# vlad17/runlmc

Hardware: AMD Instinct MI355X
Metric: kronecker_toeplitz_mvms_per_sec (higher is better)
Workload: dtype f64; 1 GPU; c5 synthetic D=10 Q=5 R=1 m=100000 (grid 100004, L=204800) N=128 probes/GPU, batch=129 vectors/step, K_UU product, kernel family rbf; kern=rbf, D=10, Q=5, m=100004, L=204800, batch=129, parallelism=probe-shard x1

## Files before the change

### runlmc_amd/csrc/rl_gridop.hip

```cpp
#include "rl_host.h"

static thread_local std::string g_err;

int fail(int code, const std::string& msg) {
    g_err = msg;
    return code;
}

extern "C" const char* rl_last_error(void) { return g_err.c_str(); }
extern "C" const char* rl_backend(void) { return RL_BACKEND_NAME; }
extern "C" int rl_abi_version(void) { return RL_ABI_VERSION; }
extern "C" int rl_device_count(int* count) {
    if (!count) return fail(RL_EINVAL, "count is NULL");
    RL_HIP(hipGetDeviceCount(count));
    return RL_OK;
}

void trace_once(const char* what) {
    static const bool on = getenv("RUNLMC_TRACE") != nullptr;
    if (!on) return;
    static std::vector<std::string> seen;
    for (const std::string& s : seen)
        if (s == what) return;
    seen.push_back(what);
    fprintf(stderr, "[runlmc] %s\n", what);
}

bool first_on_device(unsigned long long* seen) {
    int dev = 0;
    (void)hipGetDevice(&dev);
    const unsigned long long bit = 1ull << (dev & 63);
    if (*seen & bit) return false;
    *seen |= bit;
    return true;
}

RlKnobs read_knobs() {
    RlKnobs k;
    const char* dbg = getenv("RUNLMC_DEBUG");
    const bool debug = dbg != nullptr && dbg[0] != '\0' && dbg[0] != '0';
    auto ignored = [](const char* n) {
        static std::vector<std::string> told;
        if (std::find(told.begin(), told.end(), std::string(n)) == told.end()) {
            told.push_back(n);
            fprintf(stderr, "runlmc_hip: %s is a debug switch and is ignored without RUNLMC_DEBUG=1\n", n);
        }
    };
    auto user_flag = [](const char* n) { return getenv(n) != nullptr; };
    auto user_num = [](const char* n, long long dflt) {
        const char* e = getenv(n);
        return e ? atoll(e) : dflt;
    };
    auto flag = [&](const char* n) {
        if (getenv(n) == nullptr) return false;
        if (!debug) ignored(n);
        return debug;
    };
    auto num = [&](const char* n, long long dflt) {
        const char* e = getenv(n);
        if (e == nullptr) return dflt;
        if (!debug) ignored(n);
        return debug ? atoll(e) : dflt;
    };
    k.pow2_only = user_flag("RUNLMC_POW2_ONLY");
    k.chunk_mb = (int)num("RUNLMC_CHUNK_MB", 0);
    k.two_streams = (int)num("RUNLMC_TWO_STREAMS", -1);
    k.affine = (int)num("RUNLMC_AFFINE", -1);
    k.affine_kb = (int)num("RUNLMC_AFFINE_KB", 0);
    k.affine_max_kb = (int)num("RUNLMC_AFFINE_MAX_KB", 2048);
    k.no_v1p = flag("RUNLMC_NO_V1P");
    k.v1p_min = (int)num("RUNLMC_V1P_MIN", 0);
    k.no_lowrank = flag("RUNLMC_NO_LOWRANK");
    k.no_filter = flag("RUNLMC_NO_FILTER");
    k.no_lr_bound = flag("RUNLMC_NO_LR_BOUND");
    k.sf_carries1 = flag("RUNLMC_SF_CARRIES1");
    k.sf_scan2 = flag("RUNLMC_SF_SCAN2");
    k.poly_round = flag("RUNLMC_POLY_ROUND");
    k.no_poly_round = flag("RUNLMC_NO_POLY_ROUND");
    k.lr_min = num("RUNLMC_LR_MIN", -1);
    k.staged_wt = flag("RUNLMC_STAGED_WT");
    k.no_staged_wt = flag("RUNLMC_NO_STAGED_WT");
    k.no_w_poly = flag("RUNLMC_NO_W_POLY");
    k.no_rp = flag("RUNLMC_NO_RP");
    k.rp_stagger = (int)num("RUNLMC_RP_STAGGER", 7);
    k.no_lr_small = flag("RUNLMC_NO_LR_SMALL");
    k.no_precond_approx = flag("RUNLMC_NO_PRECOND_APPROX");
    k.no_precond_hi = flag("RUNLMC_NO_PRECOND_HI");
    k.precond_hi_passes = flag("RUNLMC_PRECOND_HI_PASSES");
    k.no_precond_hi_mixed = flag("RUNLMC_NO_PRECOND_HI_MIXED");
    k.precond_hi_min = num("RUNLMC_PRECOND_HI_MIN", 100000);
    k.precond_hi_rank = (int)num("RUNLMC_PRECOND_HI_RANK", 192);
    k.precond_hi_use = (int)num("RUNLMC_PRECOND_HI_USE", 0);
    k.rp_fly = (int)num("RUNLMC_RP_FLY", 1);
    k.no_rp_small = flag("RUNLMC_NO_RP_SMALL");
    k.no_rp_fuse = flag("RUNLMC_NO_RP_FUSE");
    k.rp_pfuse = !flag("RUNLMC_NO_RP_PFUSE");
    k.w_pfuse = !flag("RUNLMC_NO_W_PFUSE");
    k.rp_runlen = (int)num("RUNLMC_RP_RUNLEN", 0);
    k.w_poly_rmax = std::min(36, (int)num("RUNLMC_W_POLY_RMAX", 32));
    k.no_sort = flag("RUNLMC_NO_SORT");
    k.ws_cache_mb = user_num("RUNLMC_WS_CACHE_MB", -1);
    k.solver_maxblk = (int)num("RUNLMC_SOLVER_MAXBLK", 0);
    k.no_fuse_w = flag("RUNLMC_NO_FUSE_W");
    k.no_fuse_wt = flag("RUNLMC_NO_FUSE_WT");
    k.no_graph = flag("RUNLMC_NO_GRAPH");
#if defined(RL_EMU)
    k.minres_v1 = flag("RUNLMC_MINRES_V1");
#endif
    return k;
}

static int ilog2(int x) {
    int l = 0;
    while ((1 << l) < x) ++l;
    return l;
}

static FftPlan make_plan(int n) {
    FftPlan p;
    p.n = n;
    p.npass = 0;
    for (int i = 0; i < RL_MAX_PASSES; ++i) p.radix[i] = 1;
    int rem = n;
    for (int odd : {3, 5})
        while (rem % odd == 0 && p.npass < 2) {
            p.radix[p.npass++] = odd;
            rem /= odd;
        }
    const int fixed[7][4] = {{8, 8, 0, 0},     {16, 16, 0, 0},   {64, 8, 8, 0},
                             {128, 8, 16, 0},  {256, 16, 16, 0}, {512, 8, 8, 8},
                             {1024, 8, 8, 16}};
    for (const auto& f : fixed)
        if (f[0] == rem) {
            for (int i = 1; i < 4 && f[i]; ++i) p.radix[p.npass++] = f[i];
            return p;
        }
    while (rem > 1) {
        int r = 8;
        while (rem % r) r /= 2;
        p.radix[p.npass++] = r;
        rem /= r;
    }
    return p;
}

static bool make_plan_rows3(int n, FftPlan* p) {
    int ra, rb;
    switch (n) {
        case 128: ra = 8; rb = 8; break;
        case 256: ra = 16; rb = 8; break;
        case 512: ra = 16; rb = 16; break;
        default: return false;
    }
    p->n = n;
    p->npass = 3;
    for (int i = 0; i < RL_MAX_PASSES; ++i) p->radix[i] = 1;
    p->radix[0] = ra;
    p->radix[1] = rb;
    p->radix[2] = 2;
    return true;
}

static int fused_code(const FftPlan& p) {
    if (p.npass < 2 || p.npass > 4) return 0;
    const int ra = p.radix[0], rb = p.radix[p.npass - 1];
    const int code = ra * 100 + rb;
    switch (code) {
        case 808: case 816: case 1616: return p.n >= 64 ? code : 0;
// ... 983 lines not shown
        for (int n = 0; n < m; ++n) {
            prev[n] = cur[n];
            cur[n] = nxt[n] / bj;
        }
    }
    RL_TRY(upload(&g->lr_phiJ, phiJ));
    RL_TRY(upload(&g->lr_beta, beta));
    RL_TRY(upload(&g->lr_nu, nu));
    g->lr_hnu = nu;
    return RL_OK;
}

static int lr_steps(const rl_gridop* g, int nrows, int R) {
    const int slots = (g->m + 1) / 2;
    if (slots <= 64 * RL_LR_T) return std::max(4, ((slots + 63) / 64 + 3) / 4 * 4);
    const int rowblocks = (nrows + RL_LR_ROWS(R) - 1) / RL_LR_ROWS(R);
    const double resident = 2.0 * RL_LR_CUS;
    int best = RL_LR_T;
    double best_cost = 1e300;
    for (int steps = RL_LR_T; steps <= 8 * RL_LR_T; steps *= 2) {
        const int chunks = ((g->m + 1) / 2 + 64 * steps - 1) / (64 * steps);
        const double rounds = std::ceil((double)chunks * rowblocks / resident);
        const double cost = rounds * (steps + 8);
        if (cost < best_cost * 0.97) {
            best_cost = cost;
            best = steps;
        }
        if (chunks == 1) break;
    }
    return best;
}
static int lr_nchunks_max(const rl_gridop* g) {
    return ((g->m + 1) / 2 + 64 * RL_LR_T - 1) / (64 * RL_LR_T);
}
static size_t lr_part_need(const rl_gridop* g, int nvec) {
    return (size_t)lr_nchunks_max(g) * nvec * g->D * RL_LR_RMAX;
}
int lr_reserve(rl_gridop* g, int nvec) {
    const size_t rows = (size_t)nvec * g->D;
    const size_t need_part = lr_part_need(g, nvec), need_z = rows * RL_LR_RMAX;
    if (g->lr_part_cap < need_part) {
        if (g->lr_part) RL_HIP(hipFree(g->lr_part));
        g->lr_part = nullptr;
        g->lr_part_cap = 0;
        RL_HIP(hipMalloc((void**)&g->lr_part, need_part * sizeof(double)));
        g->lr_part_cap = need_part;
    }
    if (g->lr_zhat_cap < need_z) {
        if (g->lr_zhat) RL_HIP(hipFree(g->lr_zhat));
        g->lr_zhat = nullptr;
        g->lr_zhat_cap = 0;
        RL_HIP(hipMalloc((void**)&g->lr_zhat, need_z * sizeof(double)));
        g->lr_zhat_cap = need_z;
    }
    return RL_OK;
}

static size_t lr_min_elements(const rl_gridop* g) {
    return g->kn.lr_min >= 0 ? (size_t)g->kn.lr_min : (size_t)1 << 20;
}

template <int R>
static int lr_project(rl_gridop* g, const double* X, int nrows, hipStream_t st,
                      double* part = nullptr) {
    const int steps = lr_steps(g, nrows, R);
    const int chunks = ((g->m + 1) / 2 + 64 * steps - 1) / (64 * steps);
    RL_LAUNCH((k_lr_project<R>), dim3(chunks, (nrows + RL_LR_ROWS(R) - 1) / RL_LR_ROWS(R)),
              dim3(64 * RL_LR_WAVES), (size_t)RL_LR_WAVES * R * 65 * sizeof(double), st, X, nrows,
              g->m, (const double*)g->lr_beta, steps, part != nullptr ? part : g->lr_part);
    return chunks;
}
template <int R>
static void lr_mix(rl_gridop* g, const double* part, int chunks, int nvec, int Q, const double* Cq,
                   const double* Bq, double* zhat, hipStream_t st) {
    int split3 = 0;
    const size_t mix_lds = lr_mix_lds(g->D, R, Q, &split3);
    RL_LAUNCH(k_lr_mix, dim3(nvec), dim3(RL_LR_MIXT), mix_lds, st, part, chunks, nvec, g->D, R, Q,
              Cq, Bq, (const double*)g->lr_nu, zhat, (const int*)nullptr, split3);
}
template <int R>
static void lr_expand(rl_gridop* g, const double* zhat, int nrows, double* Y, int accumulate,
                      hipStream_t st) {
    const int per_cu = 8;
    const int nbx = ((g->m + 1) / 2 + 255) / 256;
    int rpb = 16;
    if ((size_t)nbx * ((nrows + 15) / 16) < (size_t)2 * per_cu * RL_LR_CUS) {
        const int nby = std::max(1, std::min(nrows, per_cu * RL_LR_CUS / nbx));
        rpb = (nrows + nby - 1) / nby;
    }
    if (accumulate)
        RL_LAUNCH((k_lr_expand<R, true>), dim3(nbx, (nrows + rpb - 1) / rpb), dim3(256), 0,
                  st, zhat, nrows, g->m, (const double*)g->lr_beta, rpb, Y);
    else
        RL_LAUNCH((k_lr_expand<R, false>), dim3(nbx, (nrows + rpb - 1) / rpb), dim3(256), 0,
                  st, zhat, nrows, g->m, (const double*)g->lr_beta, rpb, Y);
}
template <int R>
static void lr_launch(rl_gridop* g, const double* X, double* Y, int nvec, int Q, const double* Cq,
                      const double* Bq, hipStream_t st, int accumulate = 0) {
    const int nrows = nvec * g->D;
    const bool deferred = g->defer_expand && !accumulate && R <= g->kn.w_poly_rmax;
    const int chunks = lr_project<R>(g, X, nrows, st);
    lr_mix<R>(g, g->lr_part, chunks, nvec, Q, Cq, Bq, g->lr_zhat, st);
    if (deferred) {
        g->expand_deferred = true;
        return;
    }
    lr_expand<R>(g, g->lr_zhat, nrows, Y, accumulate, st);
}

static int lr_apply(rl_gridop* g, const double* X, double* Y, int nvec, int q0, int Q,
                    const double* Bq, hipStream_t st) {
    const double* Cq = g->lr_C + (size_t)q0 * g->lr_r * g->lr_r;
    switch (g->lr_r) {
        case 24: lr_launch<24>(g, X, Y, nvec, Q, Cq, Bq, st); break;
        case 32: lr_launch<32>(g, X, Y, nvec, Q, Cq, Bq, st); break;
        case 36: lr_launch<36>(g, X, Y, nvec, Q, Cq, Bq, st); break;
        case 40: lr_launch<40>(g, X, Y, nvec, Q, Cq, Bq, st); break;
        case 48: lr_launch<48>(g, X, Y, nvec, Q, Cq, Bq, st); break;
        default: return fail(RL_EINVAL, "low-rank path: bad basis size");
    }
    RL_HIP(hipGetLastError());
    return RL_OK;
}

static int lr_apply_compact(rl_gridop* g, const double* X, double* Y, int nvec, hipStream_t st) {
    switch (g->lr_r) {
        case 24: lr_launch<24>(g, X, Y, nvec, g->lr_np, g->lr_Cc, g->lr_Bc, st, 1); break;
        case 32: lr_launch<32>(g, X, Y, nvec, g->lr_np, g->lr_Cc, g->lr_Bc, st, 1); break;
        case 36: lr_launch<36>(g, X, Y, nvec, g->lr_np, g->lr_Cc, g->lr_Bc, st, 1); break;
        case 40: lr_launch<40>(g, X, Y, nvec, g->lr_np, g->lr_Cc, g->lr_Bc, st, 1); break;
        case 48: lr_launch<48>(g, X, Y, nvec, g->lr_np, g->lr_Cc, g->lr_Bc, st, 1); break;
        default: return fail(RL_EINVAL, "low-rank path: bad basis size");
    }
    RL_HIP(hipGetLastError());
    return RL_OK;
}

static int mvm_with_mix(rl_gridop* g, const MixParams& mp, const double* X, double* Y, int nvec,
                        hipStream_t stream);

struct SfFit {
    int deg = 0;
    long double ah = 0.0L;
    long double c[4] = {0.0L, 0.0L, 0.0L, 0.0L};
};

static bool sf_check(const double* t, int m, const SfFit& f, long double tot) {
    const long double budget = (long double)RL_SF_TOL * tot, rho = expl(-f.ah);
    long double err = 0.0L, pw = 1.0L;
    for (int i = 0; i < m; ++i) {
        if ((i & 255) == 0) pw = expl(-f.ah * i);
        const long double model = (f.c[0] + (f.c[1] + (f.c[2] + f.c[3] * i) * i) * i) * pw;
        err += fabsl((long double)t[i] - model);
        if (!(err <= budget)) return false;
        pw *= rho;
    }
    return true;
}

static bool sf_detect(const double* t, int m, SfFit* fit) {
    if (m < 8) return false;
    long double tot = 0.0L;
    double amax = 0.0;
    int imax = 0;
    for (int i = 0; i < m; ++i) {
        if (!std::isfinite(t[i])) return false;
        const double a = std::fabs(t[i]);
        tot += a;
        if (a > amax) {
            amax = a;
            imax = i;
        }
    }
    if (amax == 0.0) return false;
    int below = -1;
    for (int i = imax; i < m; ++i)
        if (std::fabs(t[i]) <= 0.6 * amax) {
// ... 1102 lines not shown
```

### runlmc_amd/csrc/rl_host.h

```cpp
#pragma once
#include "../../include/runlmc_hip.h"

#include <algorithm>
#include <cmath>
#include <cstdio>
#include <cstdlib>
#include <cstring>
#include <functional>
#include <string>
#include <thread>
#include <vector>

#include "rl_kernels.h"
#include "rl_kernels2.h"
#include "rl_kernels3.h"
#include "rl_lowrank.h"
#include "rl_rowpoly.h"
#include "rl_filter.h"

#define RL_MAX_D 16

int fail(int code, const std::string& msg);
#define RL_HIP(expr)                                                                   \
    do {                                                                               \
        hipError_t e_ = (expr);                                                        \
        if (e_ != hipSuccess)                                                          \
            return fail(RL_EHIP, std::string(#expr) + ": " + hipGetErrorString(e_));   \
    } while (0)

#define RL_TRY(expr)              \
    do {                          \
        int rc_ = (expr);         \
        if (rc_ != RL_OK) return rc_; \
    } while (0)


void trace_once(const char* what);
bool first_on_device(unsigned long long* seen);

struct RlKnobs {
    bool pow2_only = false;
    int chunk_mb = 0;
    int two_streams = -1;
    int affine = -1;
    int affine_kb = 0;
    int affine_max_kb = 2048;
    bool no_v1p = false;
    int v1p_min = 0;
    bool no_lowrank = false;
    bool no_filter = false;
    bool sf_scan2 = false;
    bool sf_carries1 = false;
    bool no_lr_bound = false;
    bool poly_round = false;
    bool no_poly_round = false;
    long long lr_min = -1;
    bool staged_wt = false;
    bool no_staged_wt = false;
    bool no_w_poly = false;
    bool no_rp = false;
    int rp_stagger = 7;
    int rp_runlen = 0;
    bool no_rp_small = false;
    bool rp_pfuse = true;
    bool w_pfuse = true;
    bool no_rp_fuse = false;
    bool no_lr_small = false;
    bool no_precond_approx = false;
    long long precond_hi_min = 100000;
    int precond_hi_use = 0;
    int precond_hi_rank = 192;
    bool no_precond_hi_mixed = false;
    bool precond_hi_passes = false;
    bool no_precond_hi = false;
    int rp_fly = 1;
    int w_poly_rmax = 32;
    bool no_sort = false;
    long long ws_cache_mb = -1;
    int solver_maxblk = 0;
    bool no_fuse_w = false;
    bool no_fuse_wt = false;
    bool no_graph = false;
    bool minres_v1 = false;
};
RlKnobs read_knobs();

template <class T>
static int upload(T** dev, const std::vector<T>& host) {
    RL_HIP(hipMalloc((void**)dev, std::max<size_t>(host.size(), 1) * sizeof(T)));
    if (!host.empty())
        RL_HIP(hipMemcpy(*dev, host.data(), host.size() * sizeof(T), hipMemcpyHostToDevice));
    return RL_OK;
}

static const size_t kLdsSoft = 76 * 1024;
static const size_t kLdsHard = 156 * 1024;

struct rl_gridop {
    RlKnobs kn;
    int device = 0;
    int D = 0, m = 0, L = 0, N1 = 0, N2 = 0;
    Geom geo{0, 0, 0};
    int colsA = 0;
    int rowsB = 0;
    int rowsS = 0;
    int code1 = 0, code2 = 0;
    bool v2 = false;
    bool rows3 = false;
    bool lr_try = false;
    bool lr_ok = false;
    bool lr_round_try = false;
    bool wide = false;
    rl_gridop* child = nullptr;
    double* wide_B = nullptr;
    double* wide_Z = nullptr;
    size_t wide_Z_cap = 0;
    bool defer_expand = false;
    bool expand_deferred = false;
    int lr_rejects = 0;
    int lr_skip = 0;
    double* lr_stat = nullptr;
    bool lr_dirty = false;
    std::vector<double> lr_A, lr_W, lr_kap;
    std::vector<int> lr_Qi;
    bool lr_bypass = false;
    int lr_r = 0;
    int lr_rank_hint = 0;
    size_t lr_min = 0;
    double* lr_beta = nullptr;
    double* lr_nu = nullptr;
    double* lr_phiJ = nullptr;
    double* lr_C = nullptr;
    double* lr_M = nullptr;
    std::vector<double> lr_hC;
    double* lr_spart = nullptr;
    size_t lr_spart_cap = 0;
    double* lr_Cx = nullptr;
    double* lr_Mf = nullptr;
    size_t lr_Mf_cap = 0;
    bool lr_Mf_ok = false;
    std::vector<double> lr_hB;
    std::vector<double> lr_hnu;
    unsigned long long param_ver = 0;
    double* lr_B = nullptr;
    double* lr_eye = nullptr;
    double* lr_part = nullptr;
    size_t lr_part_cap = 0;
    double* lr_zhat = nullptr;
    size_t lr_zhat_cap = 0;
    double* lr_scr = nullptr;
// ... 245 lines not shown
```

### runlmc_amd/csrc/rl_lowrank.h

```cpp
#pragma once
#include "rl_device.h"

#define RL_LR_RMAX 48
#define RL_LR_T 32
#define RL_LR_WAVES 4
#define RL_LR_CUS 256
#define RL_LR_RB(R) ((R) <= 24 ? 4 : 2)
#define RL_LR_G(R) ((R) <= 24 ? 2 : 4)
#define RL_LR_ROWS(R) (RL_LR_RB(R) * RL_LR_WAVES)
#if defined(RL_EMU)
#define RL_LR_PROJECT_ATTR
#define RL_LR_UNIFORM(x) (x)
#else
#define RL_LR_PROJECT_ATTR __attribute__((amdgpu_waves_per_eu(2)))
#define RL_LR_UNIFORM(x) __builtin_amdgcn_readfirstlane(x)
#endif
#define RL_LR_TOL 2e-13

__device__ __forceinline__ int lr_slots(int m) { return (m + 1) / 2; }
__device__ __forceinline__ double lr_point(int n, int m) {
    return m > 1 ? fma(2.0 / (double)(m - 1), (double)n, -1.0) : 0.0;
}

template <int R>
// ... 149 lines not shown
        const double* z = Z + b * r;
        double s = 0.0;
        for (int j = 0; j < r; ++j) s = fma(c[j], z[j], s);
        W[e] = s;
    }
    __syncthreads();
    if (!split3) {
        for (int e = tid; e < Dr; e += nthr) {
            const int a = e / r, i = e - a * r;
            double s = 0.0;
            for (int q = 0; q < Q; ++q) {
                const double* bq = Bq + ((size_t)q * D + a) * D;
                for (int b = 0; b < D; ++b) s = fma(bq[b], W[(q * D + b) * r + i], s);
            }
            Zhat[(size_t)v * Dr + e] = nu[i] * s;
        }
        return;
    }
    for (int e = tid; e < Q * Dr; e += nthr) {
        const int q = e / Dr, rem = e - q * Dr;
        const int a = rem / r, i = rem - a * r;
        const double* bq = Bq + ((size_t)q * D + a) * D;
        double s = 0.0;
        for (int b = 0; b < D; ++b) s = fma(bq[b], W[(q * D + b) * r + i], s);
        S[e] = s;
    }
    __syncthreads();
    for (int e = tid; e < Dr; e += nthr) {
        double s = 0.0;
        for (int q = 0; q < Q; ++q) s += S[q * Dr + e];
        Zhat[(size_t)v * Dr + e] = nu[e % r] * s;
    }
}

template <int R, bool ACC>
__global__ void __launch_bounds__(256)
k_lr_expand(const double* __restrict__ Zhat, int nrows, int m, const double* __restrict__ beta,
            int rows_per_block, double* __restrict__ Y) {
    const int slots = lr_slots(m);
    const int lin = blockIdx.y * gridDim.x + blockIdx.x;
    const int bx = lin / gridDim.y, by = lin - bx * gridDim.y;
    const int n = bx * 256 + threadIdx.x;
    const int nc = n < slots ? n : slots - 1;
    const int mir = m - 1 - nc;
    const bool live = n < slots, pair = live && mir != nc;
    const int row0 = by * rows_per_block;
    const int row1 = row0 + rows_per_block < nrows ? row0 + rows_per_block : nrows;
    const double s = lr_point(nc, m);
    double p[R];
    {
        double qm = 0.0, q = 1.0;
#pragma unroll
        for (int j = 0; j < R; ++j) {
            p[j] = q;
            const double qn = fma(s, q, -beta[j] * qm);
            qm = q;
            q = qn;
        }
    }
    for (int row = row0; row < row1; ++row) {
        const double* z = Zhat + (size_t)row * R;
        double zz[R];
#pragma unroll
        for (int j = 0; j < R; ++j) zz[j] = z[j];
#if !defined(RL_EMU)
        __builtin_amdgcn_sched_barrier(0);
#endif
        double ev = 0.0, od = 0.0;
#pragma unroll
        for (int j = 0; j + 1 < R; j += 2) {
            ev = fma(zz[j], p[j], ev);
            od = fma(zz[j + 1], p[j + 1], od);
        }
        double* y0 = Y + (size_t)row * m + nc;
        double* y1 = Y + (size_t)row * m + mir;
        double o0 = 0.0, o1 = 0.0;
        if constexpr (ACC) {
            o0 = *y0;
            o1 = *y1;
        }
        if (live) *y0 = (ev + od) + o0;
        if (pair) *y1 = (ev - od) + o1;
    }
}

#define RL_LR_SMALL_MAX 32768
#define RL_LR_SMALL_WG 256
#define RL_LR_SU 4
#define RL_LR_SMP 32
static inline int lr_small_nseg(int m) {
    const int slots = (m + 1) / 2;
    int nseg = (slots + RL_LR_SMALL_WG * RL_LR_SU - 1) / (RL_LR_SMALL_WG * RL_LR_SU);
    return nseg < 1 ? 1 : (nseg > 16 ? 16 : nseg);
}
template <int R>
__global__ void __launch_bounds__(RL_LR_SMALL_WG)
k_lr_small_project(const double* __restrict__ X, int D, int m, int nseg, const double* __restrict__ beta,
                   double* __restrict__ part) {
    RL_SMEM(smem);
    double* red = reinterpret_cast<double*>(smem);
    double* wsum = red + (size_t)4 * R * 65;
    const int tid = threadIdx.x, lane = tid & 63, wave = tid >> 6;
    const int b = blockIdx.x / nseg, sg = blockIdx.x - b * nseg, v = blockIdx.y;
    const int slots = lr_slots(m), seglen = (slots + nseg - 1) / nseg;
    const int n0 = sg * seglen, n1 = n0 + seglen < slots ? n0 + seglen : slots;
    const double* xb = X + ((size_t)v * D + b) * m;
    double acc[R];
#pragma unroll
    for (int j = 0; j < R; ++j) acc[j] = 0.0;
    for (int nb = n0 + tid; nb < n1; nb += RL_LR_SMALL_WG * RL_LR_SU) {
        double s[RL_LR_SU], q[RL_LR_SU], qm[RL_LR_SU], xe[RL_LR_SU], xo[RL_LR_SU];
#pragma unroll
        for (int u = 0; u < RL_LR_SU; ++u) {
            const int n = nb + RL_LR_SMALL_WG * u;
            const bool live = n < n1;
            const int nc = live ? n : n1 - 1, mir = m - 1 - nc;
            const double x0 = live ? xb[nc] : 0.0, x1 = live && mir != nc ? xb[mir] : 0.0;
            xe[u] = x0 + x1;
            xo[u] = x0 - x1;
            s[u] = lr_point(nc, m);
            q[u] = 1.0;
            qm[u] = 0.0;
        }
#pragma unroll
        for (int j = 0; j < R; ++j) {
            const double nbj = -beta[j];
#pragma unroll
            for (int u = 0; u < RL_LR_SU; ++u) {
                acc[j] = fma(q[u], (j & 1) ? xo[u] : xe[u], acc[j]);
                const double qn = fma(s[u], q[u], nbj * qm[u]);
                qm[u] = q[u];
                q[u] = qn;
            }
        }
    }
#pragma unroll
    for (int j = 0; j < R; ++j) red[((size_t)wave * R + j) * 65 + lane] = acc[j];
    __syncthreads();
    if (tid < 4 * R) {
        const double* src = red + (size_t)tid * 65;
        double s0 = 0.0, s1 = 0.0, s2 = 0.0, s3 = 0.0;
#pragma unroll 4
        for (int l = 0; l < 64; l += 4) {
            s0 += src[l];
            s1 += src[l + 1];
            s2 += src[l + 2];
            s3 += src[l + 3];
        }
        wsum[tid] = (s0 + s1) + (s2 + s3);
    }
    __syncthreads();
    if (tid < R)
        part[(((size_t)v * D + b) * nseg + sg) * R + tid] =
            (wsum[tid] + wsum[R + tid]) + (wsum[2 * R + tid] + wsum[3 * R + tid]);
}
static inline size_t lr_small_project_lds(int R) { return ((size_t)4 * R * 65 + 4 * R) * sizeof(double); }
static inline size_t lr_small_expand_lds(int D, int R) { return ((size_t)D * R + 256 + R) * sizeof(double); }

template <int R>
__global__ void __launch_bounds__(RL_LR_SMALL_WG)
k_lr_small_expand(const double* __restrict__ part, int D, int m, int nseg, const double* __restrict__ beta,
                  const double* __restrict__ Mf, double* __restrict__ Y) {
    RL_SMEM(smem);
    double* Z = reinterpret_cast<double*>(smem);
    double* P = Z + (size_t)D * R;
    double* Zh = P + 256;
// ... 259 lines not shown
```

### runlmc_amd/csrc/rl_sample.hip

```cpp
#include "rl_host.h"
#include "rl_sample.h"

#include <complex>

typedef std::complex<double> cd;

static const int kSmpTile = 4096;
static const int kSmpAxis2d = 2048;
static const long long kSmpMaxLen = 1ll << 22;

struct rl_sampler {
    rl_gridop* g = nullptr;
    int device = 0, D = 0, m = 0, m1 = 0, m2 = 0;
    bool set = false;
    int Q = 0, nemb = 0, npoly = 0, poly_rank = 0;
    long long zlen = 0;
    int N1 = 0, N2 = 0;
    bool one_launch = false;
    int cols = 1, rows = 1, K1 = 0;
    FftPlan plan1, plan2;
    cplx *tw1 = nullptr, *tw2 = nullptr, *twlo = nullptr;
    int *freq1 = nullptr, *pos1 = nullptr, *freq2 = nullptr;
    int* eC = nullptr;
    int* efoff = nullptr;
// ... 252 lines not shown
        RL_TRY(upload(&h->eC, eC));
        RL_TRY(upload(&h->efoff, efoff));
        RL_TRY(upload(&h->ezoff, ezoff));
        const int n1 = N1s, n2 = twod ? N2s : 1;
        const size_t ext_len = (size_t)(n1 / 2 + 1) * (twod ? n2 / 2 + 1 : 1);
        std::vector<double> slam((size_t)nemb * Ltot);
        h->h_lam.assign((size_t)nemb * Ltot, 0.0);
        int e = 0;
        for (int q = 0; q < Q; ++q) {
            if (forms[q] != 0) {
                if (clipped) clipped[q] = 0.0;
                continue;
            }
            const std::vector<double> lam = smp_spectrum(ext_rows + (size_t)e * ext_len, n1, n2);
            long double neg = 0.0L, tot = 0.0L;
            for (long long w = 0; w < Ltot; ++w) {
                const double v = lam[w];
                tot += std::fabs(v);
                if (v < 0.0) neg += -v;
                slam[(size_t)e * Ltot + w] = v > 0.0 ? std::sqrt(v / (double)Ltot) : 0.0;
                h->h_lam[(size_t)e * Ltot + w] = v > 0.0 ? v : 0.0;
            }
            if (clipped) clipped[q] = tot > 0.0L ? (double)(neg / tot) : 0.0;
            ++e;
        }
        RL_TRY(upload(&h->slam, slam));
        h->one_launch = !twod && Ltot <= RL_SAMPLER_LDS_MAX;
        if (h->one_launch) {
            h->N1 = (int)Ltot;
            h->N2 = 1;
        } else if (twod) {
            h->N1 = N1s;
            h->N2 = N2s;
        } else {
            int odd = 1;
            (void)smp_length_ok(Ltot, &odd);
            const long long P = Ltot / odd;
            int n2p = 1;
            while (2 * n2p <= kSmpTile && P % (2 * n2p) == 0 && Ltot / (2 * n2p) >= 16) n2p *= 2;
            h->N2 = n2p;
            h->N1 = (int)(Ltot / n2p);
            if (h->N1 > kSmpTile || h->N2 > kSmpTile || h->N1 < 1)
                return fail(RL_ELIMIT, "rl_sampler_set: embedding length has no two-pass split");
        }
        h->plan1 = smp_plan(h->N1);
        const std::vector<int> f1 = smp_pos_to_freq(h->plan1);
        RL_TRY(upload(&h->freq1, f1));
        RL_TRY(upload(&h->pos1, smp_invert(f1)));
        RL_TRY(upload(&h->tw1, smp_unity(h->N1, 1, h->N1)));
        if (!h->one_launch) {
            h->plan2 = smp_plan(h->N2);
            RL_TRY(upload(&h->freq2, smp_pos_to_freq(h->plan2)));
            RL_TRY(upload(&h->tw2, smp_unity(h->N2, 1, h->N2)));
            RL_TRY(upload(&h->twlo, smp_unity(h->N2, 1, Ltot)));
            h->cols = std::max(1, std::min(16, kSmpTile / h->N1));
            h->rows = std::max(1, std::min(16, kSmpTile / h->N2));
            while (h->rows > 1 && (long long)h->N2 * (h->rows | 1) > kSmpTile) --h->rows;
            h->K1 = twod ? h->m1 : std::min(h->N1, h->m);
        }
    }
    if (npoly) {
        RL_TRY(upload(&h->pC, pC));
        RL_TRY(upload(&h->pfoff, pfoff));
        RL_TRY(upload(&h->pzoff, pzoff));
        std::vector<double> hG(poly_sqrt, poly_sqrt + (size_t)npoly * poly_rank * poly_rank);
        RL_TRY(upload(&h->G, hG));
    }
    *zlen = h->zlen;
    h->set = true;
    return RL_OK;
}

extern "C" int rl_sampler_spectrum_host(const rl_sampler* h, int q, double* out) {
    if (!h || !out) return fail(RL_EINVAL, "rl_sampler_spectrum_host: NULL argument");
    if (!h->set || q < 0 || q >= h->Q || h->emb_of[q] < 0)
        return fail(RL_EINVAL, "rl_sampler_spectrum_host: not a row in the embedding form");
    const size_t Ltot = (size_t)h->N1 * h->N2;
    memcpy(out, h->h_lam.data() + (size_t)h->emb_of[q] * Ltot, Ltot * sizeof(double));
    return RL_OK;
}

template <int R>
static void smp_expand(rl_sampler* h, double* U, int nrows, bool accumulate, hipStream_t st) {
    const int slots = (h->m + 1) / 2, nbx = (slots + 255) / 256;
    const int nby = std::max(1, std::min(nrows, 4 * RL_LR_CUS / nbx));
    const int rpb = (nrows + nby - 1) / nby;
    const dim3 grid(nbx, (nrows + rpb - 1) / rpb);
    if (accumulate)
        RL_LAUNCH((k_lr_expand<R, true>), grid, dim3(256), 0, st, (const double*)h->zhat, nrows, h->m,
                  (const double*)h->g->lr_beta, rpb, U);
    else
        RL_LAUNCH((k_lr_expand<R, false>), grid, dim3(256), 0, st, (const double*)h->zhat, nrows, h->m,
                  (const double*)h->g->lr_beta, rpb, U);
}

extern "C" int rl_sampler_draw(rl_sampler* h, const double* Z, double* U, int nsamp, void* stream) {
    if (!h || !Z || !U) return fail(RL_EINVAL, "rl_sampler_draw: NULL argument");
    if (!h->set) return fail(RL_EINVAL, "rl_sampler_draw: no parameters (rl_sampler_set)");
    if (nsamp < 0) return fail(RL_EINVAL, "rl_sampler_draw: nsamp < 0");
    if (nsamp == 0) return RL_OK;
    const int npairs = (nsamp + 1) / 2;
    if (npairs > 65535) return fail(RL_ELIMIT, "rl_sampler_draw: at most 131070 draws per call");
    RL_HIP(hipSetDevice(h->device));
    hipStream_t st = (hipStream_t)stream;
    const int D = h->D;
    if (h->nemb) {
        SmpRows R{h->nemb, h->eC, h->efoff, h->ezoff, h->F, h->slam};
        if (h->one_launch) {
            trace_once("function draws: embedding, one launch (k_smp_embed1)");
            RL_LAUNCH(k_smp_embed1, dim3(D, npairs), dim3(RL_SMP_THREADS), (size_t)h->N1 * sizeof(cplx), st,
                      Z, h->zlen, R, D, h->m, h->plan1, (const cplx*)h->tw1, (const int*)h->pos1, U, nsamp);
        } else {
            trace_once("function draws: embedding, two passes (k_smp_cols / k_smp_rows)");
            const size_t Ltot = (size_t)h->N1 * h->N2;
            if ((size_t)npairs > h->T_pairs) {
                if (h->T) RL_HIP(hipFree(h->T));
                h->T = nullptr;
                h->T_pairs = 0;
                if (hipMalloc((void**)&h->T, (size_t)npairs * D * Ltot * sizeof(cplx)) != hipSuccess) {
                    (void)hipGetLastError();
                    return fail(RL_ENOMEM, "rl_sampler_draw: no device memory for the intermediates of " +
                                               std::to_string(npairs) + " pairs");
                }
                h->T_pairs = npairs;
            }
            const int twod = h->m1 != 0;
            RL_LAUNCH(k_smp_cols, dim3(D, (h->N2 + h->cols - 1) / h->cols, npairs), dim3(RL_SMP_THREADS),
                      (size_t)h->N1 * h->cols * sizeof(cplx), st, Z, h->zlen, R, D, h->plan1, h->N2, h->cols,
                      (const cplx*)h->tw1, (const cplx*)h->twlo, (const int*)h->freq1, twod ? 0 : 1, h->T);
            const int ld = h->rows | 1;
            RL_LAUNCH(k_smp_rows, dim3(D, (h->K1 + h->rows - 1) / h->rows, npairs), dim3(RL_SMP_THREADS),
                      (size_t)h->N2 * ld * sizeof(cplx), st, (const cplx*)h->T, D, h->N1, h->plan2, h->rows, ld,
                      h->K1, (const cplx*)h->tw2, (const int*)h->pos1, (const int*)h->freq2, h->m,
                      twod ? h->m2 : 0, U, nsamp);
        }
    }
    if (h->npoly) {
        const int r = h->poly_rank;
        if (!h->g->lr_beta || h->g->lr_r != r)
            return fail(RL_EINVAL, "rl_sampler_draw: the grid operator's polynomial form changed since rl_sampler_set");
        const size_t need = (size_t)nsamp * D * r;
        if (need > h->zhat_cap) {
            if (h->zhat) RL_HIP(hipFree(h->zhat));
            h->zhat = nullptr;
            h->zhat_cap = 0;
            RL_HIP(hipMalloc((void**)&h->zhat, need * sizeof(double)));
            h->zhat_cap = need;
        }
        trace_once("function draws: polynomial rows (k_smp_poly_coef + k_lr_expand)");
        RL_LAUNCH(k_smp_poly_coef, dim3((unsigned)((need + 255) / 256)), dim3(RL_SMP_THREADS), 0, st, Z, h->zlen,
                  h->npoly, (const int*)h->pC, (const int*)h->pfoff, (const long long*)h->pzoff,
                  (const double*)h->F, (const double*)h->G, (const double*)h->g->lr_nu, D, r, nsamp, h->zhat);
        const bool acc = h->nemb > 0;
        switch (r) {
            case 24: smp_expand<24>(h, U, nsamp * D, acc, st); break;
            case 32: smp_expand<32>(h, U, nsamp * D, acc, st); break;
            case 36: smp_expand<36>(h, U, nsamp * D, acc, st); break;
            case 40: smp_expand<40>(h, U, nsamp * D, acc, st); break;
            default: smp_expand<48>(h, U, nsamp * D, acc, st); break;
        }
    }
    RL_HIP(hipGetLastError());
    return RL_OK;
}

extern "C" int rl_normal_fill(unsigned long long seed, long long draw0, int ndraws, long long zlen,
                              double* Z, void* stream) {
    if (ndraws < 0 || zlen < 0 || draw0 < 0) return fail(RL_EINVAL, "rl_normal_fill: negative size");
    if (ndraws == 0 || zlen == 0) return RL_OK;
    if (!Z) return fail(RL_EINVAL, "rl_normal_fill: Z is NULL");
    if (ndraws > 65535) return fail(RL_ELIMIT, "rl_normal_fill: at most 65535 rows per call");
    const long long blocks = std::min<long long>((zlen + RL_SMP_THREADS - 1) / RL_SMP_THREADS, 4096);
    RL_LAUNCH(k_smp_normal, dim3((unsigned)blocks, ndraws), dim3(RL_SMP_THREADS), 0, (hipStream_t)stream, seed,
              draw0, zlen, Z);
    RL_HIP(hipGetLastError());
    return RL_OK;
// ... 16 lines not shown
```

Before: 267,600 MVM/s.

## Add alignment-phased line expand kernel for low-rank expansion writes

Adds a k_lr_expand_lines kernel that shifts each block's column window by a per-row phase, computed from the output pointer and m mod 16, so stores line up with 128-byte cache lines. Rows are grouped into classes that share the same misalignment phase. The launcher picks this kernel by default for non-accumulating expands with R<36 whenever rows are not already aligned; here m=100004 makes them unaligned. It also pads the grid y dimension to a multiple of 8 and remaps block indices. The aim is to avoid split or partial cache-line writes on the large output, at the cost of an extra block column and some idle padded blocks.

```diff
diff --git a/runlmc_amd/csrc/rl_gridop.hip b/runlmc_amd/csrc/rl_gridop.hip
--- a/runlmc_amd/csrc/rl_gridop.hip
+++ b/runlmc_amd/csrc/rl_gridop.hip
@@ -84,6 +84,7 @@
     k.no_rp = flag("RUNLMC_NO_RP");
     k.rp_stagger = (int)num("RUNLMC_RP_STAGGER", 7);
     k.no_lr_small = flag("RUNLMC_NO_LR_SMALL");
+    k.lr_expand_plain = (int)num("RUNLMC_LR_EXPAND_PLAIN", 0);
     k.no_precond_approx = flag("RUNLMC_NO_PRECOND_APPROX");
     k.no_precond_hi = flag("RUNLMC_NO_PRECOND_HI");
     k.precond_hi_passes = flag("RUNLMC_PRECOND_HI_PASSES");
@@ -1233,18 +1234,8 @@
 static void lr_expand(rl_gridop* g, const double* zhat, int nrows, double* Y, int accumulate,
                       hipStream_t st) {
     const int per_cu = 8;
-    const int nbx = ((g->m + 1) / 2 + 255) / 256;
-    int rpb = 16;
-    if ((size_t)nbx * ((nrows + 15) / 16) < (size_t)2 * per_cu * RL_LR_CUS) {
-        const int nby = std::max(1, std::min(nrows, per_cu * RL_LR_CUS / nbx));
-        rpb = (nrows + nby - 1) / nby;
-    }
-    if (accumulate)
-        RL_LAUNCH((k_lr_expand<R, true>), dim3(nbx, (nrows + rpb - 1) / rpb), dim3(256), 0,
-                  st, zhat, nrows, g->m, (const double*)g->lr_beta, rpb, Y);
-    else
-        RL_LAUNCH((k_lr_expand<R, false>), dim3(nbx, (nrows + rpb - 1) / rpb), dim3(256), 0,
-                  st, zhat, nrows, g->m, (const double*)g->lr_beta, rpb, Y);
+    lr_expand_launch<R>(zhat, nrows, g->m, (const double*)g->lr_beta, Y, accumulate != 0, 16,
+                        per_cu * RL_LR_CUS, g->kn.lr_expand_plain, st);
 }
 template <int R>
 static void lr_launch(rl_gridop* g, const double* X, double* Y, int nvec, int Q, const double* Cq,
diff --git a/runlmc_amd/csrc/rl_host.h b/runlmc_amd/csrc/rl_host.h
--- a/runlmc_amd/csrc/rl_host.h
+++ b/runlmc_amd/csrc/rl_host.h
@@ -66,6 +66,7 @@
     bool w_pfuse = true;
     bool no_rp_fuse = false;
     bool no_lr_small = false;
+    int lr_expand_plain = 0;
     bool no_precond_approx = false;
     long long precond_hi_min = 100000;
     int precond_hi_use = 0;
diff --git a/runlmc_amd/csrc/rl_lowrank.h b/runlmc_amd/csrc/rl_lowrank.h
--- a/runlmc_amd/csrc/rl_lowrank.h
+++ b/runlmc_amd/csrc/rl_lowrank.h
@@ -255,6 +255,113 @@
         if (live) *y0 = (ev + od) + o0;
         if (pair) *y1 = (ev - od) + o1;
     }
+}
+
+template <int R, bool ACC>
+__global__ void __launch_bounds__(256)
+k_lr_expand_lines(const double* __restrict__ Zhat, int nrows, int m, const double* __restrict__ beta,
+                  int rows_per_block, int period, int nby, double* __restrict__ Y) {
+    const int slots = lr_slots(m);
+    const int lin = blockIdx.y * gridDim.x + blockIdx.x;
+    const int bx = lin / gridDim.y, by = lin - bx * gridDim.y;
+    if (by >= nby) return;
+    const int cls = by % period, kb = by / period;
+    const int rfirst = cls + kb * rows_per_block * period;
+    int nr = rfirst < nrows ? (nrows - rfirst + period - 1) / period : 0;
+    nr = nr < rows_per_block ? nr : rows_per_block;
+    const int p0 = (int)((reinterpret_cast<unsigned long long>(Y) >> 3) & 15ull);
+    const int phase = (p0 + cls * (m & 15)) & 15;
+    const int n = bx * 256 + (int)threadIdx.x - phase;
+    const int nc = n < 0 ? 0 : (n < slots ? n : slots - 1);
+    const int mir = m - 1 - nc;
+    const bool live = n >= 0 && n < slots, pair = live && mir != nc;
+    const double s = lr_point(nc, m);
+    double p[R];
+    {
+        double qm = 0.0, q = 1.0;
+#pragma unroll
+        for (int j = 0; j < R; ++j) {
+            p[j] = q;
+            const double qn = fma(s, q, -beta[j] * qm);
+            qm = q;
+            q = qn;
+        }
+    }
+    for (int k = 0; k < nr; ++k) {
+        const int row = rfirst + k * period;
+        const double* z = Zhat + (size_t)row * R;
+        double zz[R];
+#pragma unroll
+        for (int j = 0; j < R; ++j) zz[j] = z[j];
+#if !defined(RL_EMU)
+        __builtin_amdgcn_sched_barrier(0);
+#endif
+        double ev = 0.0, od = 0.0;
+#pragma unroll
+        for (int j = 0; j + 1 < R; j += 2) {
+            ev = fma(zz[j], p[j], ev);
+            od = fma(zz[j + 1], p[j + 1], od);
+        }
+        double* y0 = Y + (size_t)row * m + nc;
+        double* y1 = Y + (size_t)row * m + mir;
+        double o0 = 0.0, o1 = 0.0;
+        if constexpr (ACC) {
+            o0 = *y0;
+            o1 = *y1;
+        }
+        if (live) *y0 = (ev + od) + o0;
+        if (pair) *y1 = (ev - od) + o1;
+    }
+}
+
+struct LrLinesGrid {
+    int nbx, nby, rpb, period;
+};
+static inline int lr_expand_rpb(int nbx, int nr, int ncls, int rpb_max, int round_wgs) {
+    if (rpb_max > 0 &&
+        (size_t)nbx * ncls * ((nr + rpb_max - 1) / rpb_max) >= (size_t)2 * round_wgs)
+        return rpb_max;
+    int nby = round_wgs / (nbx * ncls);
+    nby = nby < nr ? nby : nr;
+    nby = nby > 1 ? nby : 1;
+    return (nr + nby - 1) / nby;
+}
+static inline LrLinesGrid lr_expand_lines_grid(int nrows, int m, int rpb_max, int round_wgs) {
+    LrLinesGrid g;
+    int gcd = 16;
+    while ((m & 15) % gcd != 0) gcd >>= 1;
+    g.period = 16 / gcd;
+    g.nbx = ((m + 1) / 2 + 15 + 255) / 256;
+    const int ncr = (nrows + g.period - 1) / g.period;
+    g.rpb = lr_expand_rpb(g.nbx, ncr, g.period, rpb_max, round_wgs);
+    g.nby = g.period * ((ncr + g.rpb - 1) / g.rpb);
+    return g;
+}
+template <int R>
+static void lr_expand_launch(const double* zhat, int nrows, int m, const double* beta, double* Y,
+                             bool accumulate, int rpb_max, int round_wgs, int plain,
+                             hipStream_t st, bool pad8 = true) {
+    const int p0 = (int)((reinterpret_cast<unsigned long long>(Y) >> 3) & 15ull);
+    const bool measured = R < 36 && !accumulate;
+    if ((plain != 0 && plain != 3) || (plain == 0 && !measured) || ((m & 15) == 0 && p0 == 0)) {
+        const int nbx = ((m + 1) / 2 + 255) / 256;
+        const int rpb = lr_expand_rpb(nbx, nrows, 1, rpb_max, round_wgs);
+        const int nby = (nrows + rpb - 1) / rpb;
+        const dim3 grid(nbx, plain == 2 ? (nby + 7) / 8 * 8 : nby);
+        if (accumulate)
+            RL_LAUNCH((k_lr_expand<R, true>), grid, dim3(256), 0, st, zhat, nrows, m, beta, rpb, Y);
+        else
+            RL_LAUNCH((k_lr_expand<R, false>), grid, dim3(256), 0, st, zhat, nrows, m, beta, rpb, Y);
+        return;
+    }
+    const LrLinesGrid g = lr_expand_lines_grid(nrows, m, rpb_max, round_wgs);
+    const dim3 grid(g.nbx, pad8 ? (g.nby + 7) / 8 * 8 : g.nby);
+    if (accumulate)
+        RL_LAUNCH((k_lr_expand_lines<R, true>), grid, dim3(256), 0, st, zhat, nrows, m, beta, g.rpb,
+                  g.period, g.nby, Y);
+    else
+        RL_LAUNCH((k_lr_expand_lines<R, false>), grid, dim3(256), 0, st, zhat, nrows, m, beta, g.rpb,
+                  g.period, g.nby, Y);
 }
 
 #define RL_LR_SMALL_MAX 32768
diff --git a/runlmc_amd/csrc/rl_sample.hip b/runlmc_amd/csrc/rl_sample.hip
--- a/runlmc_amd/csrc/rl_sample.hip
+++ b/runlmc_amd/csrc/rl_sample.hip
@@ -358,16 +358,8 @@
 
 template <int R>
 static void smp_expand(rl_sampler* h, double* U, int nrows, bool accumulate, hipStream_t st) {
-    const int slots = (h->m + 1) / 2, nbx = (slots + 255) / 256;
-    const int nby = std::max(1, std::min(nrows, 4 * RL_LR_CUS / nbx));
-    const int rpb = (nrows + nby - 1) / nby;
-    const dim3 grid(nbx, (nrows + rpb - 1) / rpb);
-    if (accumulate)
-        RL_LAUNCH((k_lr_expand<R, true>), grid, dim3(256), 0, st, (const double*)h->zhat, nrows, h->m,
-                  (const double*)h->g->lr_beta, rpb, U);
-    else
-        RL_LAUNCH((k_lr_expand<R, false>), grid, dim3(256), 0, st, (const double*)h->zhat, nrows, h->m,
-                  (const double*)h->g->lr_beta, rpb, U);
+    lr_expand_launch<R>((const double*)h->zhat, nrows, h->m, (const double*)h->g->lr_beta, U, accumulate,
+                        0, 4 * RL_LR_CUS, h->g->kn.lr_expand_plain, st);
 }
 
 extern "C" int rl_sampler_draw(rl_sampler* h, const double* Z, double* U, int nsamp, void* stream) {
```

Result: faster. 292,800 MVM/s, median of 6 (+9.4%).
